# Rudrabha/Wav2Lip

Hardware: AMD Instinct MI355X
Metric: face-frames/sec (96x96, mel T=16) (higher is better)
Workload: dtype f32

## Files before the change

wav2lip_amd/csrc/conv_k3s.hip:

```cpp
#include "w2l_common.h"

namespace w2l {

typedef float f32x16 __attribute__((ext_vector_type(16)));
typedef float f32x4 __attribute__((ext_vector_type(4)));
typedef float f32x2 __attribute__((ext_vector_type(2)));
typedef unsigned int u32x4 __attribute__((ext_vector_type(4)));
typedef __bf16 bf16x8 __attribute__((ext_vector_type(8)));
typedef __bf16 bf16x2 __attribute__((ext_vector_type(2)));

constexpr unsigned kK3Oob = 0x80000000u;
constexpr int kK3BM = 256;
constexpr int kK3BC = 32;
constexpr int kK3KS = 16;
constexpr int kK3RP = 384;
constexpr int kK3LDY = kK3BC + 4;
constexpr int kK3KhBytes = kK3RP * 16;
constexpr int kK3PlaneBytes = 2 * kK3KhBytes;
constexpr int kK3BufBytes = 3 * kK3PlaneBytes;
constexpr int kK3StageBytes = kK3BM * kK3LDY * 4;
constexpr int kK3MainBytes = 2 * kK3BufBytes;
constexpr int kK3LdsBytes = kK3MainBytes + kK3BM * 4;
static_assert(kK3StageBytes <= kK3MainBytes && 2 * kK3LdsBytes <= 160 * 1024, "two workgroups per CU");

struct K3sKArgs {
    const void* x;
    float* y;
    uint8_t* frames;
    const float* res;
    const __bf16* u;
    const float* scale;
    const float* shift;
    const float* head_w;
    const float* head_b;
    int head_c, head_act;
    int N, H, W, cin, x_cs, y_cs, res_cs;
    int bh, bw, ni;
    int nby, nbx, ngi;
    int RH, RW, RP;
    int nkc;
    long long total;
    int act;
};

__device__ __forceinline__ unsigned k3_pack_bf16x2(float lo, float hi) {
    const f32x2 v = {lo, hi};
    return __builtin_bit_cast(unsigned, __builtin_convertvector(v, bf16x2));
}
__device__ __forceinline__ void k3_split3_pair(float x0, float x1, unsigned& h, unsigned& m, unsigned& l) {
    h = k3_pack_bf16x2(x0, x1);
    const float r0 = x0 - __uint_as_float(h << 16), r1 = x1 - __uint_as_float(h & 0xffff0000u);
    m = k3_pack_bf16x2(r0, r1);
    l = k3_pack_bf16x2(r0 - __uint_as_float(m << 16), r1 - __uint_as_float(m & 0xffff0000u));
}
__device__ __forceinline__ float k3_act(float v, int act) {
    if (act == W2L_ACT_SIGMOID) return 1.0f / (1.0f + expf(-v));
    if (act == W2L_ACT_RELU) return act_leaky(v, 0.f);
    if (act == W2L_ACT_LEAKY) return act_leaky(v, 0.01f);
    return v;
}

template <bool kBf16In, bool kU8Out>
__global__ __launch_bounds__(256, 2) void conv_k3s_kernel(const K3sKArgs a) {
    extern __shared__ __attribute__((aligned(16))) char smem[];
    int* s_opix = reinterpret_cast<int*>(smem + kK3MainBytes);
    constexpr int kEl = kBf16In ? 2 : 4;
    constexpr int kNP = kBf16In ? 1 : 3;

    const __amdgpu_buffer_rsrc_t rx = __builtin_amdgcn_make_buffer_rsrc(
        const_cast<void*>(a.x), 0, (int)((((long long)a.N * a.H * a.W - 1) * a.x_cs + a.cin) * kEl), 0x00020000);
    const int bhw = a.bh * a.bw;

    const unsigned total = (unsigned)a.total;
    const unsigned per = (total + 7u) / 8u;
    const unsigned xcd = blockIdx.x & 7u, gw = gridDim.x >> 3;
    for (unsigned jw = blockIdx.x >> 3; jw < per; jw += gw) {
    const unsigned bid = xcd * per + jw;
    if (bid >= total) break;
    int t = threadIdx.x;
    asm volatile("" : "+v"(t));
    const int lane = t & 63;
    const int wave = __builtin_amdgcn_readfirstlane(t >> 6);
    unsigned mb = bid;
    const int bx_i = (int)(mb % (unsigned)a.nbx);
    mb /= (unsigned)a.nbx;
    const int by_i = (int)(mb % (unsigned)a.nby);
    const int gi = (int)(mb / (unsigned)a.nby);

    {
        const int il = t / bhw, r = t - il * bhw;
        const int qyl = r / a.bw, qxl = r - qyl * a.bw;
        const int n = gi * a.ni + il, qy = by_i * a.bh + qyl, qx = bx_i * a.bw + qxl;
        s_opix[t] = (il < a.ni && n < a.N && qy < a.H && qx < a.W) ? (n * a.H + qy) * a.W + qx : -1;
    }

    unsigned goff[3];
    int lds_off[3];
#pragma unroll
    for (int k = 0; k < 3; ++k) {
        const int e = t + 256 * k;
        const int kh = e & 1, p = e >> 1;
        unsigned off = kK3Oob;
        if (p < a.RP) {
            const int rxx = p % a.RW, p2 = p / a.RW;
            const int ry = p2 % a.RH, il = p2 / a.RH;
            const int n = gi * a.ni + il;
            const int iy = by_i * a.bh + ry - 1, ix = bx_i * a.bw + rxx - 1;
            if (n < a.N && iy >= 0 && iy < a.H && ix >= 0 && ix < a.W)
                off = ((unsigned)((n * a.H + iy) * a.W + ix) * (unsigned)a.x_cs + (unsigned)(kh * 8)) * (unsigned)kEl;
        }
        goff[k] = off;
        lds_off[k] = kh * kK3KhBytes + p * 16;
    }
    bool slot_on[3];
#pragma unroll
    for (int k = 0; k < 3; ++k) slot_on[k] = (256 * k + wave * 64) < 2 * a.RP;
    f32x4 rawreg[3][2];
    auto raw_gload = [&](int step) {
        const unsigned soff = (unsigned)(step * kK3KS * kEl);
#pragma unroll
        for (int k = 0; k < 3; ++k) {
            if (!slot_on[k]) continue;
            rawreg[k][0] = __builtin_bit_cast(f32x4, __builtin_amdgcn_raw_buffer_load_b128(rx, (int)goff[k], (int)soff, 0));
            if constexpr (!kBf16In)
                rawreg[k][1] = __builtin_bit_cast(f32x4, __builtin_amdgcn_raw_buffer_load_b128(rx, (int)(goff[k] + 16u), (int)soff, 0));
        }
    };
    auto raw_store = [&](int buf) {
#pragma unroll
        for (int k = 0; k < 3; ++k) {
            if (!slot_on[k]) continue;
            if constexpr (kBf16In) {
                *reinterpret_cast<f32x4*>(smem + buf * kK3BufBytes + lds_off[k]) = rawreg[k][0];
                continue;
            }
            unsigned h[4], m[4], l[4];
            k3_split3_pair(rawreg[k][0][0], rawreg[k][0][1], h[0], m[0], l[0]);
            k3_split3_pair(rawreg[k][0][2], rawreg[k][0][3], h[1], m[1], l[1]);
            k3_split3_pair(rawreg[k][1][0], rawreg[k][1][1], h[2], m[2], l[2]);
            k3_split3_pair(rawreg[k][1][2], rawreg[k][1][3], h[3], m[3], l[3]);
            char* d = smem + buf * kK3BufBytes + lds_off[k];
            *reinterpret_cast<u32x4*>(d) = u32x4{h[0], h[1], h[2], h[3]};
            *reinterpret_cast<u32x4*>(d + kK3PlaneBytes) = u32x4{m[0], m[1], m[2], m[3]};
            *reinterpret_cast<u32x4*>(d + 2 * kK3PlaneBytes) = u32x4{l[0], l[1], l[2], l[3]};
        }
    };

    int abase[2];
#pragma unroll
    for (int b = 0; b < 2; ++b) {
        const int m = wave * 64 + b * 32 + (lane & 31);
        const int il = m / bhw, r = m - il * bhw;
        const int qyl = r / a.bw, qxl = r - qyl * a.bw;
        const int p = il < a.ni ? (il * a.RH + qyl) * a.RW + qxl : 0;
        abase[b] = p * 16 + (lane >> 5) * kK3KhBytes;
    }
    const int rw16 = a.RW * 16;

    const int F = a.nkc * 9 * kNP;
    const __amdgpu_buffer_rsrc_t ru = __builtin_amdgcn_make_buffer_rsrc(const_cast<__bf16*>(a.u), 0, F * 1024, 0x00020000);
    const unsigned bl_lane = (unsigned)(lane * 16);
    auto bload = [&](int kc, int tap, int plane) {
        return __builtin_bit_cast(bf16x8, __builtin_amdgcn_raw_buffer_load_b128(ru, (int)bl_lane, (int)((unsigned)((kc * 9 + tap) * kNP + plane) * 1024u), 0));
    };
    constexpr int RING = 3;
    bf16x8 bq[RING][kNP];

    f32x16 acc[2];
#pragma unroll
    for (int b = 0; b < 2; ++b)
#pragma unroll
        for (int r = 0; r < 16; ++r) acc[b][r] = 0.f;

    raw_gload(0);
#pragma unroll
    for (int i = 0; i < RING; ++i)
#pragma unroll
        for (int p = 0; p < kNP; ++p) bq[i][p] = bload(0, i, p);
    raw_store(0);
    raw_gload(1);
    __syncthreads();

    constexpr int kPa[6] = {2, 1, 0, 1, 0, 0};
    constexpr int kPb[6] = {0, 1, 2, 0, 1, 0};

    for (int step = 0; step < a.nkc; ++step) {
        const int buf = step & 1;
        raw_store(buf ^ 1);
        raw_gload(step + 2);
        const char* Ab = smem + buf * kK3BufBytes;
        bf16x8 af[2][2][kNP];
        auto aload = [&](int set, int tap) {
            const int sh = (tap / 3) * rw16 + (tap % 3) * 16;
#pragma unroll
            for (int b = 0; b < 2; ++b)
#pragma unroll
                for (int p = 0; p < kNP; ++p)
                    af[set][b][p] = *reinterpret_cast<const bf16x8*>(Ab + p * kK3PlaneBytes + abase[b] + sh);
        };
        aload(0, 0);
#pragma unroll
        for (int tap = 0; tap < 9; ++tap) {
            const int cur = tap & 1;
            if (tap + 1 < 9) aload(cur ^ 1, tap + 1);
            bf16x8 bc[kNP];
#pragma unroll
            for (int p = 0; p < kNP; ++p) bc[p] = bq[tap % RING][p];
#pragma unroll
            for (int p = 0; p < kNP; ++p)
                bq[tap % RING][p] = (tap < 6) ? bload(step, tap + 3, p) : bload(step + 1, tap - 6, p);
            __builtin_amdgcn_sched_barrier(0);
            if constexpr (kBf16In) {
#pragma unroll
                for (int b = 0; b < 2; ++b)
                    acc[b] = __builtin_amdgcn_mfma_f32_32x32x16_bf16(af[cur][b][0], bc[0], acc[b], 0, 0, 0);
            } else {
#pragma unroll
                for (int u = 0; u < 6; ++u)
#pragma unroll
                    for (int b = 0; b < 2; ++b)
                        acc[b] = __builtin_amdgcn_mfma_f32_32x32x16_bf16(af[cur][b][kPa[u]], bc[kPb[u]], acc[b], 0, 0, 0);
            }
            __builtin_amdgcn_sched_barrier(0);
        }
        __syncthreads();
    }

    float* Ys = reinterpret_cast<float*>(smem);
    {
        float* yrow = Ys + (lane & 31);
#pragma unroll
        for (int b = 0; b < 2; ++b)
#pragma unroll
            for (int r = 0; r < 16; ++r) {
                const int m = wave * 64 + b * 32 + (r & 3) + 8 * (r >> 2) + 4 * (lane >> 5);
                yrow[m * kK3LDY] = acc[b][r];
            }
    }
    __syncthreads();
    {
        const int opix = s_opix[t];
        const float* row = Ys + t * kK3LDY;
        float hacc[4] = {0.f, 0.f, 0.f, 0.f};
        if (opix >= 0) {
#pragma unroll
            for (int g = 0; g < kK3BC / 4; ++g) {
                f32x4 v = *reinterpret_cast<const f32x4*>(row + 4 * g);
                const f32x4 sc = *reinterpret_cast<const f32x4*>(a.scale + 4 * g);
                const f32x4 sh = *reinterpret_cast<const f32x4*>(a.shift + 4 * g);
                f32x4 rs = {0.f, 0.f, 0.f, 0.f};
                if (a.res) rs = *reinterpret_cast<const f32x4*>(a.res + (long long)opix * a.res_cs + 4 * g);
#pragma unroll
                for (int e = 0; e < 4; ++e) v[e] = k3_act(fmaf(v[e], sc[e], sh[e]) + rs[e], a.act);
                if (a.head_w) {
#pragma unroll
                    for (int o = 0; o < 4; ++o)
#pragma unroll
                        for (int e = 0; e < 4; ++e)
                            hacc[o] = fmaf(v[e], (o < a.head_c) ? a.head_w[o * kK3BC + 4 * g + e] : 0.f, hacc[o]);
                } else {
                    *reinterpret_cast<f32x4*>(a.y + (long long)opix * a.y_cs + 4 * g) = v;
                }
            }
            if constexpr (kU8Out) {
                for (int o = 0; o < a.head_c; ++o) {
                    const float v = k3_act(hacc[o] + (a.head_b ? a.head_b[o] : 0.f), a.head_act);
                    if (a.y) a.y[(long long)opix * a.y_cs + o] = v;
                    a.frames[(long long)opix * a.head_c + o] = (uint8_t)(int)(v * 255.0f);
                }
            } else if (a.head_w) {
                float* dst = a.y + (long long)opix * a.y_cs;
                for (int o = 0; o < a.head_c; ++o) dst[o] = k3_act(hacc[o] + (a.head_b ? a.head_b[o] : 0.f), a.head_act);
            }
        }
    }
    __syncthreads();
    }
}

struct K3sPackArgs {
    const float* w;
    __bf16* u;
    int cin;
};

template <int kNP>
__global__ void k3s_pack_kernel(const K3sPackArgs a) {
    const long long total = (long long)kK3BC * a.cin * 9;
    for (long long i = (long long)blockIdx.x * blockDim.x + threadIdx.x; i < total; i += (long long)gridDim.x * blockDim.x) {
        const int e = (int)(i & 7);
        const int ln = (int)((i >> 3) & 63);
        const long long rest = i >> 9;
        const int tap = (int)(rest % 9);
        const int kc = (int)(rest / 9);
        const int co = ln & 31, ci = kc * 16 + 8 * (ln >> 5) + e;
        const float v = a.w[((long long)co * a.cin + ci) * 9 + tap];
        const __bf16 hp = (__bf16)v;
        __bf16* d = a.u + ((long long)kc * 9 + tap) * (kNP * 512) + ln * 8 + e;
        d[0] = hp;
        if constexpr (kNP == 3) {
            const float r1 = v - (float)hp;
            const __bf16 mp = (__bf16)r1;
            d[512] = mp;
            d[1024] = (__bf16)(r1 - (float)mp);
        }
    }
}

struct K3Block { int bh, bw, ni; };
static const K3Block kK3Blocks[] = {{16, 16, 1}, {8, 16, 2}, {16, 8, 2}, {8, 8, 3}, {4, 16, 3}, {4, 8, 6}, {8, 4, 6}, {4, 4, 10}, {2, 8, 9},
                                    {2, 4, 16}, {2, 2, 24}, {1, 4, 21}, {1, 2, 32}, {1, 1, 42}, {12, 12, 1}, {6, 6, 6}, {3, 3, 15}, {8, 12, 2}};

static K3Block k3s_pick_block(int N, int H, int W) {
    K3Block best = {1, 1, 1};
    double best_cost = 1e300;
    for (const K3Block& b : kK3Blocks) {
        if (b.ni * (b.bh + 2) * (b.bw + 2) > kK3RP || b.bh * b.bw * b.ni > kK3BM) continue;
        const double items = (double)ceil_div(H, b.bh) * ceil_div(W, b.bw) * ceil_div(N, b.ni);
        const double halo = (double)(b.bh + 2) * (b.bw + 2) / ((double)b.bh * b.bw);
        const double cost = items * (1.0 + 0.03 * halo);
        if (cost < best_cost) { best_cost = cost; best = b; }
    }
    return best;
}

bool k3s_ok(const w2l_conv_geom& g) {
    return !g.transposed && g.kh == 3 && g.kw == 3 && g.sh == 1 && g.sw == 1 && g.ph == 1 && g.pw == 1 && g.cin % kK3KS == 0 &&
           g.cout == kK3BC;
}

long long k3s_u_elems(int cin) { return (long long)kK3BC * cin * 9 * 3; }
long long k3sb_u_elems(int cin) { return (long long)kK3BC * cin * 9; }

template <int kNP>
static int k3s_pack_t(const float* w, __bf16* u, int cin, hipStream_t stream) {
    K3sPackArgs pa;
    pa.w = w; pa.u = u; pa.cin = cin;
    long long blocks = ((long long)kK3BC * cin * 9 + 255) / 256;
    if (blocks > 4096) blocks = 4096;
    hipLaunchKernelGGL(k3s_pack_kernel<kNP>, dim3((unsigned)blocks), dim3(256), 0, stream, pa);
    W2L_HIP_CHECK(hipGetLastError());
    return W2L_OK;
}
int k3s_pack(const float* w, __bf16* u, int cin, hipStream_t stream) { return k3s_pack_t<3>(w, u, cin, stream); }
int k3sb_pack(const float* w, __bf16* u, int cin, hipStream_t stream) { return k3s_pack_t<1>(w, u, cin, stream); }

int k3s_init_attrs() {
    static bool done = false;
    if (done) return W2L_OK;
    W2L_HIP_CHECK(hipFuncSetAttribute(reinterpret_cast<const void*>(conv_k3s_kernel<false, false>),
                                      hipFuncAttributeMaxDynamicSharedMemorySize, kK3LdsBytes));
    done = true;
    return W2L_OK;
}

int k3sb_init_attrs() {
    static bool done = false;
    if (done) return W2L_OK;
    W2L_HIP_CHECK(hipFuncSetAttribute(reinterpret_cast<const void*>(conv_k3s_kernel<true, true>),
                                      hipFuncAttributeMaxDynamicSharedMemorySize, kK3LdsBytes));
    done = true;
    return W2L_OK;
}

void k3s_block_plan(int N, int H, int W, int out[3]) {
    const K3Block b = k3s_pick_block(N, H, W);
    out[0] = b.bh; out[1] = b.bw; out[2] = b.ni;
}

template <bool kBf16In, bool kU8Out>
static int k3s_launch_t(const void* x, int x_cs, float* y, int y_cs, uint8_t* frames, const float* res, int res_cs, const __bf16* u,
                        const float* scale, const float* shift, const float* head_w, const float* head_b, int head_c, int head_act,
                        int N, int H, int W, int cin, int act, hipStream_t stream, long long* flops_out) {
    K3sKArgs a;
    a.x = x; a.y = y; a.frames = frames; a.res = res; a.u = u; a.scale = scale; a.shift = shift;
    a.head_w = head_w; a.head_b = head_b; a.head_c = head_c; a.head_act = head_act;
    a.N = N; a.H = H; a.W = W; a.cin = cin; a.x_cs = x_cs; a.y_cs = y_cs; a.res_cs = res_cs; a.act = act;
    const K3Block b = k3s_pick_block(N, H, W);
    a.bh = b.bh; a.bw = b.bw; a.ni = b.ni;
    a.nby = ceil_div(H, b.bh);
    a.nbx = ceil_div(W, b.bw);
    a.ngi = ceil_div(N, b.ni);
    a.RH = b.bh + 2;
    a.RW = b.bw + 2;
    a.RP = b.ni * a.RH * a.RW;
    a.nkc = cin / kK3KS;
    a.total = (long long)a.ngi * a.nby * a.nbx;
    W2L_REQUIRE(a.total < (1ll << 31), "grid too large");
    W2L_REQUIRE(head_w == nullptr || (head_c >= 1 && head_c <= 4), "fused head: 1 .. 4 channels");
    if (flops_out) {
        *flops_out = (kBf16In ? 1ll : 6ll) * 2 * 9 * a.total * kK3BM * kK3BC * cin;
        return W2L_OK;
    }
    long long grid = (a.total + 7) / 8 * 8;
    if (grid > 512) grid = 512;
    hipLaunchKernelGGL((conv_k3s_kernel<kBf16In, kU8Out>), dim3((unsigned)grid), dim3(256), kK3LdsBytes, stream, a);
    W2L_HIP_CHECK(hipGetLastError());
    return W2L_OK;
}

int k3s_launch(const float* x, int x_cs, float* y, int y_cs, const float* res, int res_cs, const __bf16* u, const float* scale,
               const float* shift, const float* head_w, const float* head_b, int head_c, int head_act, int N, int H, int W, int cin,
               int act, hipStream_t stream, long long* flops_out) {
    return k3s_launch_t<false, false>(x, x_cs, y, y_cs, nullptr, res, res_cs, u, scale, shift, head_w, head_b, head_c, head_act, N, H,
                                      W, cin, act, stream, flops_out);
}

int k3sb_launch(const __bf16* x, int x_cs, uint8_t* frames, float* y, int y_cs, const __bf16* u, const float* scale, const float* shift,
                const float* head_w, const float* head_b, int head_c, int head_act, int N, int H, int W, int cin, int act,
                hipStream_t stream, long long* flops_out) {
    W2L_REQUIRE(head_w != nullptr && frames != nullptr, "k3sb: the bf16 form always runs with its head and writes uint8 frames");
    return k3s_launch_t<true, true>(x, x_cs, y, y_cs, frames, nullptr, 0, u, scale, shift, head_w, head_b, head_c, head_act, N, H, W,
                                    cin, act, stream, flops_out);
}

}
```

Before: 29460.

## Add weight-resident persistent 3x3 conv kernel for small channel counts

Adds a specialised conv kernel for cin of 16 or 32 that loads the whole packed bf16 weight set into LDS once per workgroup. The input tile for the next block is prefetched into registers while the current block's MFMAs run, so the kernel no longer streams weights through a K-loop. When the residual aliases the input, it is rebuilt from the bf16 split planes already held in LDS instead of being read again from global memory. This costs more LDS per workgroup and, for cin 32, allows only one workgroup per CU with a smaller grid cap.

```diff
diff --git a/wav2lip_amd/csrc/conv_k3s.hip b/wav2lip_amd/csrc/conv_k3s.hip
--- a/wav2lip_amd/csrc/conv_k3s.hip
+++ b/wav2lip_amd/csrc/conv_k3s.hip
@@ -6,6 +6,7 @@
 typedef float f32x4 __attribute__((ext_vector_type(4)));
 typedef float f32x2 __attribute__((ext_vector_type(2)));
 typedef unsigned int u32x4 __attribute__((ext_vector_type(4)));
+typedef unsigned int u32x2 __attribute__((ext_vector_type(2)));
 typedef __bf16 bf16x8 __attribute__((ext_vector_type(8)));
 typedef __bf16 bf16x2 __attribute__((ext_vector_type(2)));
 
@@ -41,6 +42,7 @@
     int nkc;
     long long total;
     int act;
+    int res_in_x;
 };
 
 __device__ __forceinline__ unsigned k3_pack_bf16x2(float lo, float hi) {
@@ -275,6 +277,217 @@
         }
     }
     __syncthreads();
+    }
+}
+
+constexpr int kK3WChunkBytes = 9 * 3 * 1024;
+constexpr int k3r_lds_bytes(int nkc, int rp) {
+    const int planes = rp * nkc * 16 * 6;
+    return nkc * kK3WChunkBytes + (planes > kK3StageBytes ? planes : kK3StageBytes);
+}
+static_assert(2 * k3r_lds_bytes(1, kK3RP) <= 160 * 1024 && k3r_lds_bytes(2, kK3RP) <= 160 * 1024, "LDS budget of the resident form");
+
+template <int kNKC>
+__global__ __launch_bounds__(256, kNKC == 1 ? 2 : 1) void conv_k3r_kernel(const K3sKArgs a) {
+    extern __shared__ __attribute__((aligned(16))) char smem[];
+    constexpr int kNQ = 2 * kNKC;
+    constexpr int kNS = (kK3RP * kNQ + 255) / 256;
+    char* Ws = smem;
+    char* Ps = smem + kNKC * kK3WChunkBytes;
+    const int khb = a.RP * 16;
+    const int planeb = kNQ * khb;
+
+    int t = threadIdx.x;
+    asm volatile("" : "+v"(t));
+    const int lane = t & 63;
+    const int wave = __builtin_amdgcn_readfirstlane(t >> 6);
+
+    constexpr int kWV = kNKC * kK3WChunkBytes / 16, kWN = (kWV + 255) / 256;
+    u32x4 wreg[kWN];
+#pragma unroll
+    for (int j = 0; j < kWN; ++j)
+        if (t + 256 * j < kWV) wreg[j] = *reinterpret_cast<const u32x4*>(reinterpret_cast<const char*>(a.u) + (t + 256 * j) * 16);
+
+    const __amdgpu_buffer_rsrc_t rx = __builtin_amdgcn_make_buffer_rsrc(
+        const_cast<void*>(a.x), 0, (int)((((long long)a.N * a.H * a.W - 1) * a.x_cs + a.cin) * 4), 0x00020000);
+    const int bhw = a.bh * a.bw;
+
+    int slot_pos[kNS], lds_off[kNS];
+    bool slot_on[kNS];
+#pragma unroll
+    for (int k = 0; k < kNS; ++k) {
+        const int e = t + 256 * k;
+        const int q = e % kNQ, p = e / kNQ;
+        const int rxx = p % a.RW, p2 = p / a.RW;
+        slot_pos[k] = rxx | ((p2 % a.RH) << 8) | ((p2 / a.RH) << 16);
+        slot_on[k] = p < a.RP;
+        lds_off[k] = q * khb + p * 16;
+    }
+    f32x4 rawreg[kNS][2];
+    auto raw_gload = [&](unsigned bid) {
+        unsigned mb = bid;
+        const int bx_i = (int)(mb % (unsigned)a.nbx);
+        mb /= (unsigned)a.nbx;
+        const int by_i = (int)(mb % (unsigned)a.nby);
+        const int gi = (int)(mb / (unsigned)a.nby);
+#pragma unroll
+        for (int k = 0; k < kNS; ++k) {
+            if ((256 * k + wave * 64) >= kNQ * a.RP) continue;
+            const int n = gi * a.ni + (slot_pos[k] >> 16);
+            const int iy = by_i * a.bh + ((slot_pos[k] >> 8) & 255) - 1, ix = bx_i * a.bw + (slot_pos[k] & 255) - 1;
+            unsigned off = kK3Oob;
+            if (slot_on[k] && n < a.N && iy >= 0 && iy < a.H && ix >= 0 && ix < a.W)
+                off = ((unsigned)((n * a.H + iy) * a.W + ix) * (unsigned)a.x_cs + (unsigned)(((t + 256 * k) % kNQ) * 8)) * 4u;
+            rawreg[k][0] = __builtin_bit_cast(f32x4, __builtin_amdgcn_raw_buffer_load_b128(rx, (int)off, 0, 0));
+            rawreg[k][1] = __builtin_bit_cast(f32x4, __builtin_amdgcn_raw_buffer_load_b128(rx, (int)(off + 16u), 0, 0));
+        }
+    };
+    auto raw_store = [&]() {
+#pragma unroll
+        for (int k = 0; k < kNS; ++k) {
+            if (!slot_on[k]) continue;
+            unsigned h[4], m[4], l[4];
+            k3_split3_pair(rawreg[k][0][0], rawreg[k][0][1], h[0], m[0], l[0]);
+            k3_split3_pair(rawreg[k][0][2], rawreg[k][0][3], h[1], m[1], l[1]);
+            k3_split3_pair(rawreg[k][1][0], rawreg[k][1][1], h[2], m[2], l[2]);
+            k3_split3_pair(rawreg[k][1][2], rawreg[k][1][3], h[3], m[3], l[3]);
+            char* d = Ps + lds_off[k];
+            *reinterpret_cast<u32x4*>(d) = u32x4{h[0], h[1], h[2], h[3]};
+            *reinterpret_cast<u32x4*>(d + planeb) = u32x4{m[0], m[1], m[2], m[3]};
+            *reinterpret_cast<u32x4*>(d + 2 * planeb) = u32x4{l[0], l[1], l[2], l[3]};
+        }
+    };
+
+    int abase[2];
+#pragma unroll
+    for (int b = 0; b < 2; ++b) {
+        const int m = wave * 64 + b * 32 + (lane & 31);
+        const int il = m / bhw, r = m - il * bhw;
+        const int qyl = r / a.bw, qxl = r - qyl * a.bw;
+        const int p = il < a.ni ? (il * a.RH + qyl) * a.RW + qxl : 0;
+        abase[b] = p * 16 + (lane >> 5) * khb;
+    }
+    const int rw16 = a.RW * 16;
+    const int eg = t & 7;
+    int erow[8];
+#pragma unroll
+    for (int j = 0; j < 8; ++j) {
+        const int m = (t >> 3) + 32 * j;
+        const int il = m / bhw, r = m - il * bhw;
+        const int qyl = r / a.bw;
+        erow[j] = il < a.ni ? ((r - qyl * a.bw) | (qyl << 8) | (il << 16)) : -1;
+    }
+    const f32x4 esc = *reinterpret_cast<const f32x4*>(a.scale + 4 * eg), esh = *reinterpret_cast<const f32x4*>(a.shift + 4 * eg);
+
+    constexpr int kPa[6] = {2, 1, 0, 1, 0, 0};
+    constexpr int kPb[6] = {0, 1, 2, 0, 1, 0};
+
+    const unsigned total = (unsigned)a.total;
+    const unsigned per = (total + 7u) / 8u;
+    const unsigned xcd = blockIdx.x & 7u, gw = gridDim.x >> 3;
+    unsigned jw = blockIdx.x >> 3;
+    if (jw >= per || xcd * per + jw >= total) return;
+    raw_gload(xcd * per + jw);
+#pragma unroll
+    for (int j = 0; j < kWN; ++j)
+        if (t + 256 * j < kWV) *reinterpret_cast<u32x4*>(Ws + (t + 256 * j) * 16) = wreg[j];
+    raw_store();
+    __syncthreads();
+
+    for (;;) {
+        const unsigned bid = xcd * per + jw;
+        const bool more = jw + gw < per && bid + gw < total;
+        if (more) raw_gload(bid + gw);
+
+        f32x16 acc[2];
+#pragma unroll
+        for (int b = 0; b < 2; ++b)
+#pragma unroll
+            for (int r = 0; r < 16; ++r) acc[b][r] = 0.f;
+        bf16x8 af[2][2][3], bq[2][3];
+        auto fload = [&](int set, int i) {
+            const int kc = i / 9, tap = i % 9;
+            const int sh = kc * 2 * khb + (tap / 3) * rw16 + (tap % 3) * 16;
+#pragma unroll
+            for (int p = 0; p < 3; ++p) {
+#pragma unroll
+                for (int b = 0; b < 2; ++b) af[set][b][p] = *reinterpret_cast<const bf16x8*>(Ps + p * planeb + abase[b] + sh);
+                bq[set][p] = *reinterpret_cast<const bf16x8*>(Ws + (i * 3 + p) * 1024 + lane * 16);
+            }
+        };
+        fload(0, 0);
+#pragma unroll
+        for (int i = 0; i < 9 * kNKC; ++i) {
+            const int cur = i & 1;
+            if (i + 1 < 9 * kNKC) fload(cur ^ 1, i + 1);
+            __builtin_amdgcn_sched_barrier(0);
+#pragma unroll
+            for (int u = 0; u < 6; ++u)
+#pragma unroll
+                for (int b = 0; b < 2; ++b)
+                    acc[b] = __builtin_amdgcn_mfma_f32_32x32x16_bf16(af[cur][b][kPa[u]], bq[cur][kPb[u]], acc[b], 0, 0, 0);
+            __builtin_amdgcn_sched_barrier(0);
+        }
+
+        int opix[8];
+        {
+            unsigned mb = bid;
+            const int bx_i = (int)(mb % (unsigned)a.nbx);
+            mb /= (unsigned)a.nbx;
+            const int by_i = (int)(mb % (unsigned)a.nby);
+            const int gi = (int)(mb / (unsigned)a.nby);
+#pragma unroll
+            for (int j = 0; j < 8; ++j) {
+                const int n = gi * a.ni + (erow[j] >> 16), qy = by_i * a.bh + ((erow[j] >> 8) & 255), qx = bx_i * a.bw + (erow[j] & 255);
+                opix[j] = (erow[j] >= 0 && n < a.N && qy < a.H && qx < a.W) ? (n * a.H + qy) * a.W + qx : -1;
+            }
+        }
+        const bool res_lds = kNKC == 2 && a.res_in_x;
+        f32x4 rs[8];
+        if (res_lds) {
+#pragma unroll
+            for (int j = 0; j < 8; ++j) {
+                const int cpix = erow[j] >= 0 ? ((erow[j] >> 16) * a.RH + ((erow[j] >> 8) & 255) + 1) * a.RW + (erow[j] & 255) + 1 : 0;
+                const char* s = Ps + (eg >> 1) * khb + cpix * 16 + (eg & 1) * 8;
+                const u32x2 h = *reinterpret_cast<const u32x2*>(s), m = *reinterpret_cast<const u32x2*>(s + planeb),
+                            l = *reinterpret_cast<const u32x2*>(s + 2 * planeb);
+#pragma unroll
+                for (int e = 0; e < 2; ++e) {
+                    rs[j][2 * e] = (__uint_as_float(h[e] << 16) + __uint_as_float(m[e] << 16)) + __uint_as_float(l[e] << 16);
+                    rs[j][2 * e + 1] = (__uint_as_float(h[e] & 0xffff0000u) + __uint_as_float(m[e] & 0xffff0000u)) +
+                                       __uint_as_float(l[e] & 0xffff0000u);
+                }
+            }
+        }
+        __syncthreads();
+        float* Ys = reinterpret_cast<float*>(Ps);
+        {
+            float* yrow = Ys + (lane & 31);
+#pragma unroll
+            for (int b = 0; b < 2; ++b)
+#pragma unroll
+                for (int r = 0; r < 16; ++r) {
+                    const int m = wave * 64 + b * 32 + (r & 3) + 8 * (r >> 2) + 4 * (lane >> 5);
+                    yrow[m * kK3LDY] = acc[b][r];
+                }
+        }
+        __syncthreads();
+#pragma unroll
+        for (int j = 0; j < 8; ++j) {
+            if (opix[j] < 0) continue;
+            f32x4 v = *reinterpret_cast<const f32x4*>(Ys + ((t >> 3) + 32 * j) * kK3LDY + 4 * eg);
+            f32x4 rv = {0.f, 0.f, 0.f, 0.f};
+            if (res_lds) rv = rs[j];
+            else if (a.res) rv = *reinterpret_cast<const f32x4*>(a.res + (long long)opix[j] * a.res_cs + 4 * eg);
+#pragma unroll
+            for (int e = 0; e < 4; ++e) v[e] = k3_act(fmaf(v[e], esc[e], esh[e]) + rv[e], a.act);
+            *reinterpret_cast<f32x4*>(a.y + (long long)opix[j] * a.y_cs + 4 * eg) = v;
+        }
+        if (!more) break;
+        __syncthreads();
+        raw_store();
+        __syncthreads();
+        jw += gw;
     }
 }
 
@@ -350,6 +563,10 @@
     if (done) return W2L_OK;
     W2L_HIP_CHECK(hipFuncSetAttribute(reinterpret_cast<const void*>(conv_k3s_kernel<false, false>),
                                       hipFuncAttributeMaxDynamicSharedMemorySize, kK3LdsBytes));
+    W2L_HIP_CHECK(hipFuncSetAttribute(reinterpret_cast<const void*>(conv_k3r_kernel<1>), hipFuncAttributeMaxDynamicSharedMemorySize,
+                                      k3r_lds_bytes(1, kK3RP)));
+    W2L_HIP_CHECK(hipFuncSetAttribute(reinterpret_cast<const void*>(conv_k3r_kernel<2>), hipFuncAttributeMaxDynamicSharedMemorySize,
+                                      k3r_lds_bytes(2, kK3RP)));
     done = true;
     return W2L_OK;
 }
@@ -376,6 +593,7 @@
     a.x = x; a.y = y; a.frames = frames; a.res = res; a.u = u; a.scale = scale; a.shift = shift;
     a.head_w = head_w; a.head_b = head_b; a.head_c = head_c; a.head_act = head_act;
     a.N = N; a.H = H; a.W = W; a.cin = cin; a.x_cs = x_cs; a.y_cs = y_cs; a.res_cs = res_cs; a.act = act;
+    a.res_in_x = 0;
     const K3Block b = k3s_pick_block(N, H, W);
     a.bh = b.bh; a.bw = b.bw; a.ni = b.ni;
     a.nby = ceil_div(H, b.bh);
@@ -393,6 +611,19 @@
         return W2L_OK;
     }
     long long grid = (a.total + 7) / 8 * 8;
+    if constexpr (!kBf16In) {
+        if (head_w == nullptr && (cin == 16 || cin == 32)) {
+            a.res_in_x = (cin == kK3BC && res != nullptr && static_cast<const void*>(res) == x && res_cs == x_cs) ? 1 : 0;
+            const long long cap = cin == 16 ? 512 : 256;
+            if (grid > cap) grid = cap;
+            if (cin == 16)
+                hipLaunchKernelGGL(conv_k3r_kernel<1>, dim3((unsigned)grid), dim3(256), k3r_lds_bytes(1, a.RP), stream, a);
+            else
+                hipLaunchKernelGGL(conv_k3r_kernel<2>, dim3((unsigned)grid), dim3(256), k3r_lds_bytes(2, a.RP), stream, a);
+            W2L_HIP_CHECK(hipGetLastError());
+            return W2L_OK;
+        }
+    }
     if (grid > 512) grid = 512;
     hipLaunchKernelGGL((conv_k3s_kernel<kBf16In, kU8Out>), dim3((unsigned)grid), dim3(256), kK3LdsBytes, stream, a);
     W2L_HIP_CHECK(hipGetLastError());
```

Result: no change. 29340 (-0.4%).
